# UM-ARM-Lab/pytorch_volumetric

Measured on AMD Instinct MI355X. Metric: SDF (val+grad) queries/sec, higher is better.
Workload: dtype f32

## Files before the change

pytorch_volumetric_amd/csrc/mesh.hip:

```cpp
#include "common.h"
#include "mesh_math.h"
#include "mesh_records.h"
#include "morton.h"
#include "order_small.h"
#include "wave_ops.h"

namespace pvamd {


struct MeshArgs {
    const float* normal;
    const float* rec;
    const float* tiles;
    const int* rec_of_face;
    int F;
    double ray_dir[3];
    unsigned long long* pairs;
};
#define PVAMD_COUNT_PAIRS(m, which, n)                                                                                  \
    do {                                                                                                                \
        if ((m).pairs) {                                                                                                \
            const unsigned long long count_ = (unsigned long long)(n);  \
            if ((int)(threadIdx.x & 63) == __builtin_ctzll(__ballot(true))) atomicAdd((m).pairs + (which), count_);     \
        }                                                                                                               \
// ... 94 lines not shown
        sx += __shfl_xor(sx, off, 64); sy += __shfl_xor(sy, off, 64);
        sz += __shfl_xor(sz, off, 64); sn += __shfl_xor(sn, off, 64);
    }
    if (lane == 0) { sh[wave][0] = sx; sh[wave][1] = sy; sh[wave][2] = sz; sh[wave][3] = sn; }
    __syncthreads();
    const float tn = sh[0][3] + sh[1][3] + sh[2][3] + sh[3][3];
    const float mx = (sh[0][0] + sh[1][0] + sh[2][0] + sh[3][0]) / tn;
    const float my = (sh[0][1] + sh[1][1] + sh[2][1] + sh[3][1]) / tn;
    const float mz = (sh[0][2] + sh[1][2] + sh[2][2] + sh[3][2]) / tn;
    __syncthreads();
    float reach = 0.f;
    if (live) {
        const float dx = cx - mx, dy = cy - my, dz = cz - mz;
        reach = sqrt_rn(dx * dx + dy * dy + dz * dz) * 1.00001f + r;
    }
    for (int off = 32; off > 0; off >>= 1) reach = fmaxf(reach, __shfl_xor(reach, off, 64));
    if (lane == 0) sh[wave][0] = reach;
    __syncthreads();
    if (threadIdx.x == 0) {
        float* w = tiles + 4 * (int64_t)tile;
        w[0] = mx; w[1] = my; w[2] = mz;
        w[3] = fmaxf(fmaxf(sh[0][0], sh[1][0]), fmaxf(sh[2][0], sh[3][0])) * 1.00001f + abs_margin;
    }
}

PVAMD_DEV float norm3_unfused(V3 g) {
    return sqrt_rn(add_rn(add_rn(mul_rn(g.x, g.x), mul_rn(g.y, g.y)), mul_rn(g.z, g.z)));
}

struct LaneState {
    V3 p;
    float reach;
    float reach2m, reach2x;
};

PVAMD_DEV void set_reach(LaneState& s, float reach) {
    s.reach = reach;
    s.reach2m = reach * reach * 1.00001f;
    s.reach2x = 2.00002f * reach;
}

PVAMD_DEV bool sphere_may_improve(const LaneState& s, float dist2, float r) {
    return !(dist2 > fmaf(r, fmaf(r, 1.00001f, s.reach2x), s.reach2m));
}

PVAMD_DEV bool sphere_may_hit(float dist2, float tp, float r) {
    const float perp2 = fmaf(-tp, tp, dist2);
    return !(perp2 > fmaf(r, r, 2e-6f * dist2)) && !(tp < -r);
}

PVAMD_DEV bool rect_may_improve(const LaneState& s, V3 w, float dist2, V3 fu, float hu, V3 fv, float hv, float m0) {
    const float u = dot(fu, w), v = dot(fv, w);
    const float h2 = fmaxf(fmaf(-v, v, fmaf(-u, u, dist2)), 0.f);
    const float du = fmaxf(fabsf(u) - hu, 0.f), dv = fmaxf(fabsf(v) - hv, 0.f);
    const float lb2 = fmaf(dv, dv, fmaf(du, du, h2));
    return !(lb2 > fmaf(8e-6f, dist2, s.reach2m + m0));
}

constexpr int kQueueCap = 128;
constexpr unsigned long long kBestInit = 0x7F80000000000000ull;

template <bool WITH_RAY>
struct WaveLocal {
    f32x4 sphere[64], fu[64], fv[64];
    float m0[64];
    unsigned qc[kQueueCap];
    unsigned qr[WITH_RAY ? kQueueCap : 1];
};
template <bool WITH_RAY>
struct GroupShared {
    unsigned long long best[64];
    int hits[WITH_RAY ? 64 : 1];
    int handed;
    float dir[WITH_RAY ? 192 : 1];
    float dn[WITH_RAY ? 192 : 1];
};
template <int SLICES, bool WITH_RAY>
struct MeshShared {
    GroupShared<WITH_RAY> g;
    WaveLocal<WITH_RAY> w[SLICES];
};

PVAMD_DEV float uniform(float v) { return __int_as_float(__builtin_amdgcn_readfirstlane(__float_as_int(v))); }

struct WaveBound {
    LaneState q;
    float rho;
    V3 dn0;
    float k, rho_k;
};

template <bool WITH_RAY>
struct Wave {
    LaneState s;
    bool live;
    V3 dn, dir;
    WaveBound wb;
    int nc, nr;
};

template <bool WITH_RAY>
PVAMD_DEV void refresh_bound(Wave<WITH_RAY>& wv) {
    const float rmax = wave_max(wv.live ? wv.s.reach : 0.f);
    set_reach(wv.wb.q, uniform((rmax + wv.wb.rho) * 1.00001f));
}

template <bool WITH_RAY>
PVAMD_DEV void pull_reach(const GroupShared<WITH_RAY>& g, Wave<WITH_RAY>& wv) {
    const float d2 = __int_as_float((int)(unsigned)(g.best[threadIdx.x & 63] >> 32));
    const float reach = fast_sqrt(d2) * 1.00001f + 1.1e-19f;
    if (reach < wv.s.reach) set_reach(wv.s, reach);
    refresh_bound(wv);
}

template <bool WITH_RAY>
PVAMD_DEV bool wave_setup(const MeshArgs& m, Wave<WITH_RAY>& wv) {
    const V3 p = wv.s.p;
    wv.live = fabsf(p.x) < INFINITY && fabsf(p.y) < INFINITY && fabsf(p.z) < INFINITY;
    wv.nc = wv.nr = 0;
    set_reach(wv.s, INFINITY);
    if (__ballot(wv.live) == 0ull) return false;
    const float lx = wave_min(wv.live ? p.x : INFINITY), hx = wave_max(wv.live ? p.x : -INFINITY);
    const float ly = wave_min(wv.live ? p.y : INFINITY), hy = wave_max(wv.live ? p.y : -INFINITY);
    const float lz = wave_min(wv.live ? p.z : INFINITY), hz = wave_max(wv.live ? p.z : -INFINITY);
    wv.wb.q.p = v3(uniform(0.5f * lx + 0.5f * hx), uniform(0.5f * ly + 0.5f * hy), uniform(0.5f * lz + 0.5f * hz));
    const V3 d = v3(p.x - wv.wb.q.p.x, p.y - wv.wb.q.p.y, p.z - wv.wb.q.p.z);
    wv.wb.rho = uniform(wave_max(wv.live ? fast_sqrt(dot(d, d)) : 0.f) * 1.00001f + 1.1e-19f);
    wv.wb.dn0 = v3(0.f, 0.f, 0.f);
    wv.wb.k = wv.wb.rho_k = 0.f;
    if (WITH_RAY) {
        const V3 a = v3((float)m.ray_dir[0], (float)m.ray_dir[1], (float)m.ray_dir[2]);
        const float inv = 1.f / sqrt_rn(dot(a, a));
        wv.wb.dn0 = v3(uniform(a.x * inv), uniform(a.y * inv), uniform(a.z * inv));
        const V3 e = v3(wv.dn.x - wv.wb.dn0.x, wv.dn.y - wv.wb.dn0.y, wv.dn.z - wv.wb.dn0.z);
        const float chord = wave_max(wv.live ? fast_sqrt(dot(e, e)) : 0.f);
        wv.wb.k = uniform(2.001f * chord + 2e-6f);
        wv.wb.rho_k = uniform(wv.wb.rho * (1.f + wv.wb.k) * 1.00001f);
    }
    set_reach(wv.wb.q, INFINITY);
    return true;
}

PVAMD_DEV bool axis_may_hit(const WaveBound& wb, V3 w, float dist2, float r) {
    const float dist = fast_sqrt(dist2) * 1.00001f + 1.1e-19f;
    return sphere_may_hit(dist2, dot(w, wb.dn0), fmaf(wb.k, dist, r + wb.rho_k));
}

PVAMD_DEV void enqueue(unsigned* q, int& n, unsigned long long mask, bool mine, int j) {
    const int lane = threadIdx.x & 63;
    if (mine) q[n + __popcll(mask & ((1ull << lane) - 1ull))] = ((unsigned)j << 6) | (unsigned)lane;
    n += __popcll(mask);
}

template <class Fn>
PVAMD_DEV void drain(unsigned* q, int& n, bool everything, Fn&& fn) {
    const int lane = threadIdx.x & 63;
    PVAMD_WAVE_SYNC();
    fn(n < 64 ? n : 64, q);
    if (n > 64) {
        const int rem = n - 64;
        if (everything) {
            fn(rem, q + 64);
            n = 0;
        } else {
            const unsigned v = lane < rem ? q[64 + lane] : 0u;
            if (lane < rem) q[lane] = v;
            n = rem;
        }
    } else {
        n = 0;
    }
    PVAMD_WAVE_SYNC();
}

template <bool WITH_RAY>
PVAMD_DEV void drain_closest(const MeshArgs& m, GroupShared<WITH_RAY>& g, WaveLocal<WITH_RAY>& wl, Wave<WITH_RAY>& wv, bool everything) {
    if (wv.nc == 0) return;
    const int lane = threadIdx.x & 63;
    drain(wl.qc, wv.nc, everything, [&](int count, const unsigned* q) {
        PVAMD_COUNT_PAIRS(m, 0, count);
        const unsigned e = lane < count ? q[lane] : 0u;
        const int owner = e & 63;
        const V3 p = v3(__shfl(wv.s.p.x, owner, 64), __shfl(wv.s.p.y, owner, 64), __shfl(wv.s.p.z, owner, 64));
        if (lane < count) {
            const int j = (int)(e >> 6);
            const f32x4 A = record_plane(m.rec, j, kPlaneA), B = record_plane(m.rec, j, kPlaneB), C = record_plane(m.rec, j, kPlaneC);
            const V3 qp = sub(closest_point_triangle(p, xyz(A), xyz(B), xyz(C)), p);
            const float d2 = dot(qp, qp);
            atomicMin(&g.best[owner], ((unsigned long long)(unsigned)__float_as_int(d2) << 32) | (unsigned)__float_as_int(A.w));
        }
    });
    pull_reach(g, wv);
}

template <bool WITH_RAY>
PVAMD_DEV void drain_rays(const MeshArgs& m, GroupShared<WITH_RAY>& g, WaveLocal<WITH_RAY>& wl, Wave<WITH_RAY>& wv, bool everything) {
    if (wv.nr == 0) return;
    const int lane = threadIdx.x & 63;
    drain(wl.qr, wv.nr, everything, [&](int count, const unsigned* q) {
        PVAMD_COUNT_PAIRS(m, 1, count);
        const unsigned e = lane < count ? q[lane] : 0u;
        const int owner = e & 63;
        const V3 p = v3(__shfl(wv.s.p.x, owner, 64), __shfl(wv.s.p.y, owner, 64), __shfl(wv.s.p.z, owner, 64));
        const V3 d = v3(__shfl(wv.dir.x, owner, 64), __shfl(wv.dir.y, owner, 64), __shfl(wv.dir.z, owner, 64));
        if (lane < count) {
            const int j = (int)(e >> 6);
            const f32x4 A = record_plane(m.rec, j, kPlaneA), B = record_plane(m.rec, j, kPlaneB), C = record_plane(m.rec, j, kPlaneC);
            if (ray_hits_triangle(p, d, xyz(A), xyz(B), xyz(C))) atomicAdd(&g.hits[owner], 1);
        }
    });
}

template <bool WITH_RAY>
PVAMD_DEV void visit_tile(const MeshArgs& m, GroupShared<WITH_RAY>& g, WaveLocal<WITH_RAY>& wl, Wave<WITH_RAY>& wv, int ti,
                          int pass_lo = 0, int pass_hi = kTile / 64) {
    const int lane = threadIdx.x & 63;
    const int ntiles = (m.F + kTile - 1) / kTile;
    const int n = min(kTile, m.F - ti * kTile);
    unsigned gm = 0u;
    {
        const bool gv = lane < kGroupsPerTile && lane * kGroup < n;
        const f32x4 gs = reinterpret_cast<const f32x4*>(m.tiles)[ntiles + ti * kGroupsPerTile + (gv ? lane : 0)];
        const V3 wc = v3(gs.x - wv.wb.q.p.x, gs.y - wv.wb.q.p.y, gs.z - wv.wb.q.p.z);
        const float dc2 = dot(wc, wc);
        bool coarse = sphere_may_improve(wv.wb.q, dc2, gs.w);
        if (WITH_RAY) coarse = coarse || axis_may_hit(wv.wb, wc, dc2, gs.w);
        unsigned todo = (unsigned)__ballot(coarse && gv);
        todo &= ((1u << (pass_hi * (64 / kGroup))) - 1u) & ~((1u << (pass_lo * (64 / kGroup))) - 1u);
        while (todo != 0u) {
            const int b = __builtin_ctz(todo);
            todo &= todo - 1u;
            const V3 ctr = v3(__int_as_float(__builtin_amdgcn_readlane(__float_as_int(gs.x), b)),
                              __int_as_float(__builtin_amdgcn_readlane(__float_as_int(gs.y), b)),
                              __int_as_float(__builtin_amdgcn_readlane(__float_as_int(gs.z), b)));
            const float r = __int_as_float(__builtin_amdgcn_readlane(__float_as_int(gs.w), b));
            const V3 w = v3(ctr.x - wv.s.p.x, ctr.y - wv.s.p.y, ctr.z - wv.s.p.z);
            const float dist2 = dot(w, w);
            bool need = sphere_may_improve(wv.s, dist2, r);
            if (WITH_RAY) need = need || sphere_may_hit(dist2, dot(w, wv.dn), r);
            if (__ballot(need && wv.live) != 0ull) gm |= 1u << b;
        }
    }
    const f32x4* P0 = tile_plane(m.rec, ti, kPlaneSphere);
    const f32x4* P1 = tile_plane(m.rec, ti, kPlaneU);
    const f32x4* P2 = tile_plane(m.rec, ti, kPlaneV);
    const f32x4* P4 = tile_plane(m.rec, ti, kPlaneB);
    for (int pass = pass_lo; pass < pass_hi; ++pass) {
        if (((gm >> (pass * (64 / kGroup))) & ((1u << (64 / kGroup)) - 1u)) == 0u) continue;
        const int idx = pass * 64 + lane;
        const f32x4 a0 = P0[idx], a1 = P1[idx], a2 = P2[idx];
        const float am0 = P4[idx].w;
        bool keep_c, keep_r = false;
        {
            const bool valid = idx < n && ((gm >> (idx / kGroup)) & 1u);
            const V3 w = v3(a0.x - wv.wb.q.p.x, a0.y - wv.wb.q.p.y, a0.z - wv.wb.q.p.z);
            const float dist2 = dot(w, w);
            keep_c = valid && sphere_may_improve(wv.wb.q, dist2, a0.w) &&
                     rect_may_improve(wv.wb.q, w, dist2, xyz(a1), a1.w, xyz(a2), a2.w, am0);
            if (WITH_RAY) keep_r = valid && axis_may_hit(wv.wb, w, dist2, a0.w);
        }
        const unsigned long long mc = __ballot(keep_c), mr = WITH_RAY ? __ballot(keep_r) : 0ull;
        unsigned long long todo = mc | mr;
        if (todo == 0ull) continue;
        PVAMD_WAVE_SYNC();
        wl.sphere[lane] = a0;
        wl.fu[lane] = a1;
        wl.fv[lane] = a2;
        wl.m0[lane] = am0;
        PVAMD_WAVE_SYNC();
        const int j0 = ti * kTile + pass * 64;
        const unsigned long long live_mask = __ballot(wv.live);
        while (todo != 0ull) {
            const int b = __builtin_ctzll(todo);
            todo &= todo - 1ull;
            const f32x4 o = wl.sphere[b];
            const V3 w = v3(o.x - wv.s.p.x, o.y - wv.s.p.y, o.z - wv.s.p.z);
            const float dist2 = dot(w, w);
            if (!WITH_RAY || ((mc >> b) & 1ull)) {
                const unsigned long long near_c = live_mask & __ballot(sphere_may_improve(wv.s, dist2, o.w));
                if (near_c != 0ull) {
                    const f32x4 u = wl.fu[b], v = wl.fv[b];
                    const unsigned long long mk = near_c & __ballot(rect_may_improve(wv.s, w, dist2, xyz(u), u.w, xyz(v), v.w, wl.m0[b]));
                    if (mk) {
                        enqueue(wl.qc, wv.nc, mk, __builtin_amdgcn_inverse_ballot_w64(mk), j0 + b);
                        if (wv.nc >= 64) drain_closest(m, g, wl, wv, false);
                    }
                }
            }
            if (WITH_RAY && ((mr >> b) & 1ull)) {
                const unsigned long long mk = live_mask & __ballot(sphere_may_hit(dist2, dot(w, wv.dn), o.w));
                if (mk) {
                    enqueue(wl.qr, wv.nr, mk, __builtin_amdgcn_inverse_ballot_w64(mk), j0 + b);
                    if (wv.nr >= 64) drain_rays(m, g, wl, wv, false);
                }
            }
        }
    }
}

template <bool WITH_RAY>
PVAMD_DEV int scan_seed(const MeshArgs& m, Wave<WITH_RAY>& wv, int part, int nparts) {
    const int lane = threadIdx.x & 63;
    const int ntiles = (m.F + kTile - 1) / kTile;
    const f32x4* tiles4 = reinterpret_cast<const f32x4*>(m.tiles);
    float bound = INFINITY, own = INFINITY;
    int nearest = -1;
    for (int base = 0; base < ntiles; base += 64) {
        const int ti = base + lane;
        if (ti < ntiles) {
            const f32x4 ts = tiles4[ti];
            const V3 w = v3(ts.x - wv.wb.q.p.x, ts.y - wv.wb.q.p.y, ts.z - wv.wb.q.p.z);
            const float b = fast_sqrt(dot(w, w)) * 1.00001f + (ts.w + 1.1e-19f);
            bound = fminf(bound, b);
            if ((nparts == 1 || (ti % nparts) == part) && (b < own || nearest < 0)) {
                own = b < own ? b : own;
                nearest = ti;
            }
        }
    }
    const float lowest = wave_min(bound);
    set_reach(wv.s, (lowest + wv.wb.rho) * 1.00001f);
    refresh_bound(wv);
    const float mine = wave_min(own);
    unsigned long long at = __ballot(nearest >= 0 && own == mine);
    if (at == 0ull) at = __ballot(nearest >= 0);
    return at ? __builtin_amdgcn_readlane(nearest, __builtin_ctzll(at)) : -1;
}

template <bool WITH_RAY>
PVAMD_DEV void greedy_reach(const MeshArgs& m, GroupShared<WITH_RAY>& g, Wave<WITH_RAY>& wv, int ti) {
    const int ntiles = (m.F + kTile - 1) / kTile;
    const f32x4* spheres = reinterpret_cast<const f32x4*>(m.tiles);
    const V3 p = wv.s.p;
    auto reach_of = [&](f32x4 sp) {
        const V3 w = v3(sp.x - p.x, sp.y - p.y, sp.z - p.z);
        return fast_sqrt(dot(w, w)) * 1.00001f + (sp.w + 1.1e-19f);
    };
    float bound = INFINITY;
    int gi = 0;
    const int ngroups = (min(kTile, m.F - ti * kTile) + kGroup - 1) / kGroup;
    for (int k = 0; k < ngroups; ++k) {
        const float b = reach_of(spheres[ntiles + ti * kGroupsPerTile + k]);
        if (b < bound) { bound = b; gi = k; }
    }
    const int j0 = ti * kTile + gi * kGroup;
    float nearest = INFINITY;
    int jn = -1;
    for (int k = 0; k < kGroup; ++k) {
        if (j0 + k < m.F) {
            const float b = reach_of(record_plane(m.rec, j0 + k, kPlaneSphere));
            if (b < nearest) { nearest = b; jn = j0 + k; }
        }
    }
    PVAMD_COUNT_PAIRS(m, 0, __popcll(__ballot(jn >= 0 && wv.live)));
    if (jn >= 0 && wv.live) {
        const f32x4 A = record_plane(m.rec, jn, kPlaneA), B = record_plane(m.rec, jn, kPlaneB), C = record_plane(m.rec, jn, kPlaneC);
        const V3 qp = sub(closest_point_triangle(p, xyz(A), xyz(B), xyz(C)), p);
        const float d2 = dot(qp, qp);
        atomicMin(&g.best[threadIdx.x & 63], ((unsigned long long)(unsigned)__float_as_int(d2) << 32) | (unsigned)__float_as_int(A.w));
    }
    bound = fminf(bound, nearest) * 1.00001f;
    if (bound < wv.s.reach) set_reach(wv.s, bound);
    pull_reach(g, wv);
}

template <bool WITH_RAY>
PVAMD_DEV void scan_tiles(const MeshArgs& m, GroupShared<WITH_RAY>& g, WaveLocal<WITH_RAY>& wl, Wave<WITH_RAY>& wv, int skip,
                          int part, int nparts, int pass_lo = 0, int pass_hi = kTile / 64) {
    const int lane = threadIdx.x & 63;
    const int ntiles = (m.F + kTile - 1) / kTile;
    const f32x4* tiles4 = reinterpret_cast<const f32x4*>(m.tiles);
    for (int base = 0; base < ntiles; base += 64) {
        const int ti = base + lane;
        const bool mine = ti < ntiles && ti != skip && (nparts == 1 || (ti % nparts) == part);
        const f32x4 ts = tiles4[mine ? ti : 0];
        const V3 w = v3(ts.x - wv.wb.q.p.x, ts.y - wv.wb.q.p.y, ts.z - wv.wb.q.p.z);
        const float dist2 = dot(w, w);
        const bool ray = WITH_RAY && mine && axis_may_hit(wv.wb, w, dist2, ts.w);
        const float lower = mine ? fast_sqrt(dist2) - ts.w : INFINITY;
        unsigned long long done = 0ull;
        for (;;) {
            pull_reach(g, wv);
            const bool need = mine && (ray || sphere_may_improve(wv.wb.q, dist2, ts.w));
            const unsigned long long todo = __ballot(need) & ~done;
            if (todo == 0ull) break;
            const float key = ((todo >> lane) & 1ull) ? lower : INFINITY;
            const unsigned long long at = __ballot(key == wave_min(key)) & todo;
            const int t = __builtin_ctzll(at ? at : todo);
            done |= 1ull << t;
            const V3 ctr = v3(__int_as_float(__builtin_amdgcn_readlane(__float_as_int(ts.x), t)),
                              __int_as_float(__builtin_amdgcn_readlane(__float_as_int(ts.y), t)),
                              __int_as_float(__builtin_amdgcn_readlane(__float_as_int(ts.z), t)));
            const float r = __int_as_float(__builtin_amdgcn_readlane(__float_as_int(ts.w), t));
            const V3 wl_ = v3(ctr.x - wv.s.p.x, ctr.y - wv.s.p.y, ctr.z - wv.s.p.z);
            const float d2 = dot(wl_, wl_);
            bool mine_too = sphere_may_improve(wv.s, d2, r);
            if (WITH_RAY) mine_too = mine_too || sphere_may_hit(d2, dot(wl_, wv.dn), r);
            if (__ballot(mine_too && wv.live) == 0ull) continue;
            visit_tile<WITH_RAY>(m, g, wl, wv, base + t, pass_lo, pass_hi);
        }
    }
}

template <bool WITH_RAY>
PVAMD_DEV void scan_finish(const MeshArgs& m, GroupShared<WITH_RAY>& g, WaveLocal<WITH_RAY>& wl, Wave<WITH_RAY>& wv) {
    drain_closest(m, g, wl, wv, true);
    if (WITH_RAY) drain_rays(m, g, wl, wv, true);
}

template <bool WITH_RAY>
PVAMD_DEV bool scan_begin(const MeshArgs& m, GroupShared<WITH_RAY>& g, Wave<WITH_RAY>& wv, int wave, uint64_t seed,
                          int64_t jitter_index, const unsigned long long* start, const float* __restrict__ drawn = nullptr,
                          const float* __restrict__ bound = nullptr) {
    const int lane = threadIdx.x & 63;
    if (wave == 0) {
        g.best[lane] = start ? *start : kBestInit;
        if (WITH_RAY) {
            g.hits[lane] = 0;
            const V3 dir = drawn ? v3(drawn[3 * lane], drawn[3 * lane + 1], drawn[3 * lane + 2])
                                 : jitter_dir(m.ray_dir, seed, jitter_index);
            const float inv_len = 1.f / sqrt_rn(dot(dir, dir));
            g.dir[3 * lane] = dir.x; g.dir[3 * lane + 1] = dir.y; g.dir[3 * lane + 2] = dir.z;
            g.dn[3 * lane] = dir.x * inv_len; g.dn[3 * lane + 1] = dir.y * inv_len; g.dn[3 * lane + 2] = dir.z * inv_len;
        }
    }
    __syncthreads();
    wv.dir = wv.dn = v3(0.f, 0.f, 0.f);
    if (WITH_RAY) {
        wv.dir = v3(g.dir[3 * lane], g.dir[3 * lane + 1], g.dir[3 * lane + 2]);
        wv.dn = v3(g.dn[3 * lane], g.dn[3 * lane + 1], g.dn[3 * lane + 2]);
    }
    return bound ? load_bound(bound, wv) : wave_setup(m, wv);
}

struct HandOver {
    int* count;
    int* entries;
    unsigned long long* best;
    int* hits;
    float* dir;
    float* reach;
    float* pts;
    unsigned long long* p_best;
    float* p_dir;
    float* p_reach;
    float* bound;
    int cap;
};
constexpr int kBoundFloats = 16;
constexpr int kSmallPoints = PVAMD_MESH_SMALL_POINTS;
static_assert(PVAMD_MESH_SMALL_POINTS <= kOrderSmallPoints, "an unordered query is sorted by ONE workgroup (order_small_block), which drops the points beyond its capacity");
constexpr int kHandOverHeader = 64;
struct HandOverLayout {
    size_t entries, best, hits, dir, reach, bound, pts;
    size_t p_best, p_dir, p_reach;
    size_t bytes;
};
constexpr HandOverLayout hand_over_layout(int64_t cap) {
    const size_t slots = (size_t)cap, lanes = slots * 64, small = (size_t)kSmallPoints;
    HandOverLayout l = {};
    l.entries = kHandOverHeader;
    l.best = l.entries + slots * 2 * sizeof(int);
    l.hits = l.best + lanes * sizeof(unsigned long long);
    l.dir = l.hits + lanes * sizeof(int);
    l.reach = l.dir + lanes * 3 * sizeof(float);
    l.bound = l.reach + lanes * sizeof(float);
    l.pts = l.bound + slots * kBoundFloats * sizeof(float);
    l.p_best = l.pts + lanes * 3 * sizeof(float);
    l.p_dir = l.p_best + small * sizeof(unsigned long long);
    l.p_reach = l.p_dir + small * 3 * sizeof(float);
    l.bytes = l.p_reach + small * sizeof(float);
    return l;
}
static_assert(hand_over_layout(PVAMD_MESH_SCRATCH_SLOTS(0)).bytes == PVAMD_MESH_SCRATCH_BYTES(0) &&
              hand_over_layout(PVAMD_MESH_SCRATCH_SLOTS(1)).bytes == PVAMD_MESH_SCRATCH_BYTES(1),
              "PVAMD_MESH_SCRATCH_BYTES is not the hand-over layout's total");
static_assert(hand_over_layout(0).bytes - hand_over_layout(0).p_best == (size_t)kSmallPoints * (sizeof(unsigned long long) + 4 * sizeof(float)),
              "the by-point part holds one (best, dir, reach) per point of the largest unordered query");

static HandOver hand_over(void* scratch, int cap) {
    const HandOverLayout l = hand_over_layout(cap);
    char* base = reinterpret_cast<char*>(scratch);
    HandOver h;
    h.count = reinterpret_cast<int*>(base);
    h.entries = reinterpret_cast<int*>(base + l.entries);
    h.best = reinterpret_cast<unsigned long long*>(base + l.best);
    h.hits = reinterpret_cast<int*>(base + l.hits);
    h.dir = reinterpret_cast<float*>(base + l.dir);
    h.reach = reinterpret_cast<float*>(base + l.reach);
    h.bound = reinterpret_cast<float*>(base + l.bound);
    h.pts = reinterpret_cast<float*>(base + l.pts);
    h.p_best = reinterpret_cast<unsigned long long*>(base + l.p_best);
    h.p_dir = reinterpret_cast<float*>(base + l.p_dir);
    h.p_reach = reinterpret_cast<float*>(base + l.p_reach);
    h.cap = scratch ? cap : 0;
    return h;
}
constexpr int kHeavy32nds = 6;
constexpr int kHeavyMinTiles = 128;
constexpr int kHeavyParts = 32;

PVAMD_DEV void store_bound(float* __restrict__ b, const WaveBound& wb, bool any_live) {
    if ((threadIdx.x & 63) != 0) return;
    b[0] = wb.q.p.x; b[1] = wb.q.p.y; b[2] = wb.q.p.z; b[3] = wb.rho;
    b[4] = wb.dn0.x; b[5] = wb.dn0.y; b[6] = wb.dn0.z; b[7] = wb.k;
    b[8] = wb.rho_k; b[9] = any_live ? 1.f : 0.f;
    b[10] = wb.q.reach;
}
template <bool WITH_RAY>
PVAMD_DEV bool part_has_work(const MeshArgs& m, const float* __restrict__ b, int part, int nparts) {
    if (uniform(b[9]) == 0.f) return false;
    WaveBound wb;
    wb.q.p = v3(uniform(b[0]), uniform(b[1]), uniform(b[2]));
    wb.rho = uniform(b[3]);
    wb.dn0 = v3(uniform(b[4]), uniform(b[5]), uniform(b[6]));
    wb.k = uniform(b[7]);
    wb.rho_k = uniform(b[8]);
    set_reach(wb.q, uniform(b[10]));
    const int lane = threadIdx.x & 63;
    const int ntiles = (m.F + kTile - 1) / kTile;
    const f32x4* tiles4 = reinterpret_cast<const f32x4*>(m.tiles);
    for (int base = part; base < ntiles; base += 64 * nparts) {
        const int ti = base + lane * nparts;
        const f32x4 ts = tiles4[ti < ntiles ? ti : 0];
        const V3 w = v3(ts.x - wb.q.p.x, ts.y - wb.q.p.y, ts.z - wb.q.p.z);
        const float dist2 = dot(w, w);
        bool need = sphere_may_improve(wb.q, dist2, ts.w);
        if (WITH_RAY) need = need || axis_may_hit(wb, w, dist2, ts.w);
        if (__ballot(need && ti < ntiles) != 0ull) return true;
    }
    return false;
}
template <bool WITH_RAY>
PVAMD_DEV bool load_bound(const float* __restrict__ b, Wave<WITH_RAY>& wv) {
    const V3 p = wv.s.p;
    wv.live = fabsf(p.x) < INFINITY && fabsf(p.y) < INFINITY && fabsf(p.z) < INFINITY;
    wv.nc = wv.nr = 0;
    set_reach(wv.s, INFINITY);
    wv.wb.q.p = v3(uniform(b[0]), uniform(b[1]), uniform(b[2]));
    wv.wb.rho = uniform(b[3]);
    wv.wb.dn0 = v3(uniform(b[4]), uniform(b[5]), uniform(b[6]));
    wv.wb.k = uniform(b[7]);
    wv.wb.rho_k = uniform(b[8]);
    set_reach(wv.wb.q, INFINITY);
    return uniform(b[9]) != 0.f;
}

template <bool WITH_RAY>
PVAMD_DEV int flagged_tiles(const MeshArgs& m, const Wave<WITH_RAY>& wv) {
    const int lane = threadIdx.x & 63;
    const int ntiles = (m.F + kTile - 1) / kTile;
    const f32x4* tiles4 = reinterpret_cast<const f32x4*>(m.tiles);
// ... 182 lines not shown
    const int ntiles = (m.F + kTile - 1) / kTile;
    const f32x4* spheres = reinterpret_cast<const f32x4*>(m.tiles);
    auto reach_of = [&](f32x4 sp) {
        const V3 w = v3(sp.x - p.x, sp.y - p.y, sp.z - p.z);
        return fast_sqrt(dot(w, w)) * 1.00001f + (sp.w + 1.1e-19f);
    };
    int ti = 0;
    for (int base = 0; base < ntiles; base += 64) {
        const f32x4 mine = spheres[base + lane < ntiles ? base + lane : base];
        const int n = min(64, ntiles - base);
        for (int t = 0; t < n; ++t) {
            const f32x4 sp = {__int_as_float(__builtin_amdgcn_readlane(__float_as_int(mine.x), t)),
                              __int_as_float(__builtin_amdgcn_readlane(__float_as_int(mine.y), t)),
                              __int_as_float(__builtin_amdgcn_readlane(__float_as_int(mine.z), t)),
                              __int_as_float(__builtin_amdgcn_readlane(__float_as_int(mine.w), t))};
            const float b = reach_of(sp);
            if (b < bound) { bound = b; ti = base + t; }
        }
    }
    int gi = 0;
    const int ngroups = (min(kTile, m.F - ti * kTile) + kGroup - 1) / kGroup;
    for (int k = 0; k < kGroupsPerTile; ++k) {
        if (k >= ngroups) break;
        const float b = reach_of(spheres[ntiles + ti * kGroupsPerTile + k]);
        if (b < bound) { bound = b; gi = k; }
    }
    const int j0 = ti * kTile + gi * kGroup;
    float nearest = INFINITY;
    int jn = -1;
    for (int k = 0; k < kGroup; ++k) {
        if (j0 + k >= m.F) break;
        const float b = reach_of(record_plane(m.rec, j0 + k, kPlaneSphere));
        if (b < nearest) { nearest = b; jn = j0 + k; }
    }
    bound = fminf(bound, nearest);
    PVAMD_COUNT_PAIRS(m, 0, __popcll(__ballot(jn >= 0 && fabsf(p.x) < INFINITY && fabsf(p.y) < INFINITY && fabsf(p.z) < INFINITY)));
    if (jn >= 0 && fabsf(p.x) < INFINITY && fabsf(p.y) < INFINITY && fabsf(p.z) < INFINITY) {
        const f32x4 A = record_plane(m.rec, jn, kPlaneA), B = record_plane(m.rec, jn, kPlaneB), C = record_plane(m.rec, jn, kPlaneC);
        const V3 qp = sub(closest_point_triangle(p, xyz(A), xyz(B), xyz(C)), p);
        const float d2 = dot(qp, qp);
        found = ((unsigned long long)(unsigned)__float_as_int(d2) << 32) | (unsigned)__float_as_int(A.w);
        if (!(found < kBestInit)) found = kBestInit;
        else bound = fminf(bound, fast_sqrt(d2) * 1.00001f + 1.1e-19f);
    }
    return bound * 1.00001f;
}

__global__ __launch_bounds__(128) void hand_over_all_kernel(MeshArgs m, const int* __restrict__ order, const float* __restrict__ pts,
                                                            int64_t P, uint64_t seed, int64_t index_base, HandOver ho, int groups) {
    __shared__ float reach_of_lane[64];
    const int g = blockIdx.x, lane = threadIdx.x & 63;
    const int64_t slot = (int64_t)g * 64 + lane;
    const int64_t i = point_index(order, slot, P);
    if (threadIdx.x < 64) {
        ho.hits[slot] = 0;
        const V3 dir = jitter_dir(m.ray_dir, seed, index_base + i);
        float* o = ho.dir + slot * 3;
        o[0] = dir.x; o[1] = dir.y; o[2] = dir.z;
        {
            Wave<true> wv{};
            wv.s.p = v3(pts[3 * i], pts[3 * i + 1], pts[3 * i + 2]);
            const float inv_len = 1.f / sqrt_rn(dot(dir, dir));
            wv.dir = dir;
            wv.dn = v3(dir.x * inv_len, dir.y * inv_len, dir.z * inv_len);
            const bool any_live = wave_setup(m, wv);
            float* q = ho.pts + slot * 3;
            q[0] = wv.s.p.x; q[1] = wv.s.p.y; q[2] = wv.s.p.z;
            if (lane == 0) {
                ho.entries[2 * g] = g;
                ho.entries[2 * g + 1] = 0;
                if (g == 0) *ho.count = groups;
            }
            __syncthreads();
            if (any_live) {
                set_reach(wv.s, reach_of_lane[lane]);
                refresh_bound(wv);
            }
            store_bound(ho.bound + (int64_t)g * kBoundFloats, wv.wb, any_live);
        }
        return;
    }
    unsigned long long found;
    const float bound = greedy_bound(m, v3(pts[3 * i], pts[3 * i + 1], pts[3 * i + 2]), found);
    ho.best[slot] = found;
    ho.reach[slot] = bound;
    reach_of_lane[lane] = bound;
    __syncthreads();
}
__global__ void hand_over_none_kernel(HandOver ho) { *ho.count = 0; }

constexpr int kPrepPoints = 512;
static unsigned small_prep_blocks(int64_t P) { return 1 + (unsigned)((P + kPrepPoints - 1) / kPrepPoints); }
static_assert(kOrderSmallThreads == 1024 && kPrepPoints * 2 == kOrderSmallThreads,
              "mesh_small_prep_kernel: block 0 runs order_small_block, the others 512 points on two halves of 1024 threads");
__global__ __launch_bounds__(1024) void mesh_small_prep_kernel(MeshArgs m, const float* __restrict__ pts, int P, uint64_t seed,
                                                               int64_t index_base, int* __restrict__ order, HandOver ho) {
    if (blockIdx.x == 0) {
        order_small_block(pts, P, order, nullptr, nullptr);
        return;
    }
    const int wave = threadIdx.x >> 6, lane = threadIdx.x & 63;
    const int i = ((int)blockIdx.x - 1) * kPrepPoints + (wave & 7) * 64 + lane;
    const int ii = i < P ? i : P - 1;
    if (((int)blockIdx.x - 1) * kPrepPoints + (wave & 7) * 64 >= P) return;
    if (wave < 8) {
        const V3 dir = jitter_dir(m.ray_dir, seed, index_base + ii);
        if (i < P) {
            float* o = ho.p_dir + 3 * (int64_t)i;
            o[0] = dir.x; o[1] = dir.y; o[2] = dir.z;
        }
    } else {
        unsigned long long found;
        const float bound = greedy_bound(m, v3(pts[3 * ii], pts[3 * ii + 1], pts[3 * ii + 2]), found);
        if (i < P) {
            ho.p_best[i] = found;
            ho.p_reach[i] = bound;
        }
    }
}

__global__ __launch_bounds__(64) void hand_over_gather_kernel(MeshArgs m, const int* __restrict__ order, const float* __restrict__ pts,
                                                              int64_t P, HandOver ho, int groups) {
    const int g = blockIdx.x, lane = threadIdx.x;
    const int64_t slot = (int64_t)g * 64 + lane;
    const int64_t i = point_index(order, slot, P);
    const V3 dir = v3(ho.p_dir[3 * i], ho.p_dir[3 * i + 1], ho.p_dir[3 * i + 2]);
    const float reach = ho.p_reach[i];
    ho.best[slot] = ho.p_best[i];
    ho.reach[slot] = reach;
    ho.hits[slot] = 0;
    float* o = ho.dir + slot * 3;
    o[0] = dir.x; o[1] = dir.y; o[2] = dir.z;
    Wave<true> wv{};
    wv.s.p = v3(pts[3 * i], pts[3 * i + 1], pts[3 * i + 2]);
    float* q = ho.pts + slot * 3;
    q[0] = wv.s.p.x; q[1] = wv.s.p.y; q[2] = wv.s.p.z;
    const float inv_len = 1.f / sqrt_rn(dot(dir, dir));
    wv.dir = dir;
    wv.dn = v3(dir.x * inv_len, dir.y * inv_len, dir.z * inv_len);
    const bool any_live = wave_setup(m, wv);
    if (any_live) {
        set_reach(wv.s, reach);
        refresh_bound(wv);
    }
    store_bound(ho.bound + (int64_t)g * kBoundFloats, wv.wb, any_live);
    if (lane == 0) {
        ho.entries[2 * g] = g;
        ho.entries[2 * g + 1] = 0;
        if (g == 0) *ho.count = groups;
    }
}

constexpr int kPartsMinWaves = 7;
template <bool WITH_RAY, bool WAIT = false, int WAVES = kTile / 64>
PVAMD_DEV void parts_of_group(const MeshArgs& m, MeshShared<WAVES, WITH_RAY>& sh, uint64_t seed, const HandOver& ho, int slot) {
    const int lane = threadIdx.x & 63, wave = __builtin_amdgcn_readfirstlane(threadIdx.x >> 6);
    if (!part_has_work<WITH_RAY>(m, ho.bound + (int64_t)slot * kBoundFloats, (int)blockIdx.y, (int)gridDim.y)) return;
    Wave<WITH_RAY> wv;
    const float* q = ho.pts + ((int64_t)slot * 64 + lane) * 3;
    wv.s.p = v3(q[0], q[1], q[2]);
    const unsigned long long start = ho.best[(int64_t)slot * 64 + lane];
    const float known = ho.reach[(int64_t)slot * 64 + lane];
    if (scan_begin(m, sh.g, wv, wave, seed, 0, &start, WITH_RAY ? ho.dir + (int64_t)slot * 192 : nullptr,
                   ho.bound + (int64_t)slot * kBoundFloats)) {
        if (__any(wv.live && !(known < INFINITY) && (unsigned)(start >> 32) >= 0x7F800000u)) scan_seed(m, wv, 0, 1);
        if (known < wv.s.reach) set_reach(wv.s, known);
        refresh_bound(wv);
        constexpr int kPasses = (kTile / 64) / WAVES;
        scan_tiles<WITH_RAY>(m, sh.g, sh.w[wave], wv, -1, (int)blockIdx.y, (int)gridDim.y, wave * kPasses, (wave + 1) * kPasses);
        scan_finish(m, sh.g, sh.w[wave], wv);
    }
    __syncthreads();
    if (wave == 0) {
        if (WAIT) {
            unsigned long long was = 0ull;
            int had = 0;
            if (sh.g.best[lane] < start) was = atomicMin(&ho.best[(int64_t)slot * 64 + lane], sh.g.best[lane]);
            if (WITH_RAY && sh.g.hits[lane] != 0) had = atomicAdd(&ho.hits[(int64_t)slot * 64 + lane], sh.g.hits[lane]);
            asm volatile("" ::"v"(was), "v"(had) : "memory");
        } else {
            if (sh.g.best[lane] < start) atomicMin(&ho.best[(int64_t)slot * 64 + lane], sh.g.best[lane]);
            if (WITH_RAY && sh.g.hits[lane] != 0) atomicAdd(&ho.hits[(int64_t)slot * 64 + lane], sh.g.hits[lane]);
        }
    }
}

template <int kAllWaves>
__global__ __launch_bounds__(64 * kAllWaves, kPartsMinWaves) void mesh_parts_all_kernel(MeshArgs m, const int* __restrict__ order,
                                                                          const float* __restrict__ pts, int64_t P,
                                                                          uint64_t seed, HandOver ho, QueryOut out) {
    __shared__ __attribute__((aligned(16))) MeshShared<kAllWaves, true> sh;
    const int g = (int)blockIdx.x;
    parts_of_group<true, true, kAllWaves>(m, sh, seed, ho, g);
    if (threadIdx.x >= 64) return;
    const int lane = threadIdx.x;
    int done = 0;
    if (lane == 0) done = atomicAdd(&ho.entries[2 * g + 1], 1);
    if (__builtin_amdgcn_readfirstlane(done) != (int)gridDim.y - 1) return;
    const int64_t k = (int64_t)g * 64 + lane;
    if (k >= P) return;
    const int64_t i = order ? (int64_t)order[k] : k;
    const unsigned long long found = atomicMin(&ho.best[k], ~0ull);
    const int hits = atomicOr(&ho.hits[k], 0);
    write_query(m, out, i, v3(pts[3 * i], pts[3 * i + 1], pts[3 * i + 2]), found, hits);
}

template <bool WITH_RAY, int WAVES>
__global__ __launch_bounds__(64 * WAVES, kPartsMinWaves) void mesh_parts_kernel(MeshArgs m, uint64_t seed, HandOver ho) {
    __shared__ __attribute__((aligned(16))) MeshShared<WAVES, WITH_RAY> sh;
    const int listed = min(*ho.count, ho.cap);
    for (int slot = blockIdx.x; slot < listed; slot += gridDim.x) {
        parts_of_group<WITH_RAY, false, WAVES>(m, sh, seed, ho, slot);
        __syncthreads();
    }
}

__global__ __launch_bounds__(64) void mesh_query_finish_kernel(MeshArgs m, const int* __restrict__ order,
                                                               const float* __restrict__ pts, int64_t P, HandOver ho,
                                                               QueryOut out) {
    const int listed = min(*ho.count, ho.cap);
    for (int slot = blockIdx.x; slot < listed; slot += gridDim.x) {
        const int64_t k = (int64_t)ho.entries[2 * slot] * 64 + threadIdx.x;
        if (k >= P) continue;
        const int64_t i = order ? (int64_t)order[k] : k;
        write_query(m, out, i, v3(pts[3 * i], pts[3 * i + 1], pts[3 * i + 2]), ho.best[(int64_t)slot * 64 + threadIdx.x],
                    ho.hits[(int64_t)slot * 64 + threadIdx.x]);
    }
}

__global__ __launch_bounds__(64) void chamfer_finish_kernel(MeshArgs m, const int* __restrict__ order, const float* __restrict__ W,
                                                            const float* __restrict__ pts, int64_t N, float scale, HandOver ho,
                                                            double* __restrict__ out_sum, int64_t per) {
    const int listed = min(*ho.count, ho.cap);
    for (int slot = blockIdx.x; slot < listed; slot += gridDim.x) {
        const int64_t k = (int64_t)ho.entries[2 * slot] * 64 + threadIdx.x;
        const int b = ho.entries[2 * slot + 1];
        const int64_t i = point_index(order, k, N);
        const V3 p = W ? chamfer_point(W + 16 * (int64_t)b, pts, i) : v3(pts[3 * i], pts[3 * i + 1], pts[3 * i + 2]);
        chamfer_accumulate(m, p, k < N, ho.best[(int64_t)slot * 64 + threadIdx.x], scale, W ? out_sum + b : out_sum, i, W ? 0 : per);
    }
}

__global__ __launch_bounds__(256) void morton_keys_kernel(const float* __restrict__ pts, int64_t P,
                                                          const float* __restrict__ box, int* __restrict__ keys) {
    const int64_t i = (int64_t)blockIdx.x * blockDim.x + threadIdx.x;
    if (i >= P) return;
    const float lo[3] = {box[0], box[1], box[2]}, hi[3] = {box[3], box[4], box[5]};
    keys[i] = (int)morton_key30(pts[3 * i], pts[3 * i + 1], pts[3 * i + 2], lo, hi);
}

__global__ void aabb_init_kernel(unsigned* box) {
    if (threadIdx.x < 3) box[threadIdx.x] = order_code(INFINITY);
    else if (threadIdx.x < 6) box[threadIdx.x] = order_code(-INFINITY);
}
__global__ __launch_bounds__(256) void aabb_reduce_kernel(const float* __restrict__ pts, int64_t P, unsigned* box) {
    float lo[3] = {INFINITY, INFINITY, INFINITY}, hi[3] = {-INFINITY, -INFINITY, -INFINITY};
    for (int64_t i = (int64_t)blockIdx.x * blockDim.x + threadIdx.x; i < P; i += (int64_t)gridDim.x * blockDim.x) {
#pragma unroll
        for (int d = 0; d < 3; ++d) {
            const float v = pts[3 * i + d];
            if (fabsf(v) < INFINITY) {
                lo[d] = fminf(lo[d], v);
                hi[d] = fmaxf(hi[d], v);
            }
        }
    }
#pragma unroll
    for (int d = 0; d < 3; ++d) {
        for (int off = 32; off > 0; off >>= 1) {
            lo[d] = fminf(lo[d], __shfl_xor(lo[d], off, 64));
            hi[d] = fmaxf(hi[d], __shfl_xor(hi[d], off, 64));
        }
    }
    __shared__ float part[4][6];
    const int wave = threadIdx.x >> 6, lane = threadIdx.x & 63;
    if (lane == 0) {
#pragma unroll
        for (int d = 0; d < 3; ++d) { part[wave][d] = lo[d]; part[wave][3 + d] = hi[d]; }
    }
    __syncthreads();
    if (threadIdx.x < 3) {
        const int d = threadIdx.x;
        atomicMin(box + d, order_code(fminf(fminf(part[0][d], part[1][d]), fminf(part[2][d], part[3][d]))));
    } else if (threadIdx.x < 6) {
        const int d = threadIdx.x;
        atomicMax(box + d, order_code(fmaxf(fmaxf(part[0][d], part[1][d]), fmaxf(part[2][d], part[3][d]))));
    }
}
__global__ void aabb_decode_kernel(unsigned* box) {
    if (threadIdx.x < 6) reinterpret_cast<float*>(box)[threadIdx.x] = order_decode(box[threadIdx.x]);
}

__global__ void zero_f64_kernel(double* p, int n) {
    const int i = blockIdx.x * blockDim.x + threadIdx.x;
    if (i < n) p[i] = 0.0;
}

__global__ void invert_face_order_kernel(const float* __restrict__ rec, int F, int* __restrict__ rec_of_face) {
    const int k = blockIdx.x * blockDim.x + threadIdx.x;
    if (k < F) rec_of_face[__float_as_int(record_plane(rec, k, kPlaneA).w)] = k;
}

static MeshArgs mesh_args(const pvamd_mesh_t& mesh) {
    MeshArgs m;
    m.normal = mesh.normal;
    m.rec = mesh.rec;
    m.tiles = mesh.tiles;
    m.rec_of_face = mesh.rec_of_face;
    m.F = mesh.F;
    for (int d = 0; d < 3; ++d) m.ray_dir[d] = mesh.ray_dir[d];
    m.pairs = reinterpret_cast<unsigned long long*>(mesh.pair_counters);
    return m;
}

constexpr int kMaxFaces = 1 << 26;

__global__ __launch_bounds__(256) void grid_points_kernel(const float* __restrict__ cx, const float* __restrict__ cy,
                                                          const float* __restrict__ cz, int nx, int ny, int nz,
                                                          float* __restrict__ pts, int* __restrict__ order) {
    const int64_t n = (int64_t)nx * ny * nz;
    const int64_t i = (int64_t)blockIdx.x * blockDim.x + threadIdx.x;
    if (i >= n) return;
    const int z = (int)(i % nz), y = (int)((i / nz) % ny), x = (int)(i / ((int64_t)nz * ny));
    pts[3 * i] = cx[x];
    pts[3 * i + 1] = cy[y];
    pts[3 * i + 2] = cz[z];
    const int Bx = x >> 4, By = y >> 4, Bz = z >> 4;
    const int Wx = min(16, nx - 16 * Bx), Wy = min(16, ny - 16 * By), Wz = min(16, nz - 16 * Bz);
    const int sx = x & 15, sy = y & 15, sz = z & 15;
    const int bx = sx >> 2, by = sy >> 2, bz = sz >> 2;
    const int wx = min(4, Wx - 4 * bx), wy = min(4, Wy - 4 * by), wz = min(4, Wz - 4 * bz);
    const int64_t j = (int64_t)(16 * Bx) * ny * nz + (int64_t)Wx * (16 * By) * nz + (int64_t)Wx * Wy * (16 * Bz) +
                      ((int64_t)(4 * bx) * Wy * Wz + (int64_t)wx * (4 * by) * Wz + (int64_t)wx * wy * (4 * bz)) +
                      ((int64_t)((sx & 3) * wy + (sy & 3)) * wz + (sz & 3));
    order[j] = (int)i;
}

using MeshPlan = pvamd_mesh_plan_t;
constexpr int kMaxSlices = 8;
constexpr int kMinParts = 4;
constexpr int kHeavyPartWaves = 4;
constexpr int kWideScanOverTiles = 128;

static int scan_waves_for(int64_t groups, int ntiles, bool hands_over) {
    int s = 2;
    while (s < 8 && (int64_t)s * groups < 16384) s <<= 1;
    if (ntiles > kWideScanOverTiles && !hands_over) s = 8;
    if (s > kMaxSlices) s = kMaxSlices;
    while (s > 1 && s > ntiles) s >>= 1;
    return s;
}

static void plan_scan(MeshPlan& pl, int64_t rows, int ntiles, bool has_scratch) {
    const bool hands_over = has_scratch && ntiles >= kHeavyMinTiles;
    pl.path = hands_over ? PVAMD_MESH_PATH_SCAN_HEAVY : PVAMD_MESH_PATH_SCAN;
    pl.scan_waves = scan_waves_for(pl.groups * rows, ntiles, hands_over);
    pl.parts = hands_over ? (kHeavyParts < ntiles ? kHeavyParts : ntiles) : 0;
    pl.part_waves = hands_over ? kHeavyPartWaves : 0;
}

static MeshPlan mesh_query_plan(int64_t P, int F, bool has_scratch, bool unordered) {
    MeshPlan pl = {};
    const int64_t groups = (P + 63) / 64;
    const int ntiles = (F + kTile - 1) / kTile;
    pl.groups = (int32_t)groups;
// ... 227 lines not shown
```

Baseline: 213.2 billion.

## Add point-serial traversal mode for tile passes in mesh_parts_kernel

Adds a POINT_SERIAL variant of visit_tile. When few query points want a tile pass compared with the number of surviving triangles, it loops over those points and tests all triangles in parallel across lanes, instead of looping over triangles and testing all points. Candidate records are enqueued with the point index so the existing closest-point and ray drains can process them. The mode is enabled only in mesh_parts_kernel and adds extra ballots and readlanes per point in exchange for better lane utilisation when points are sparse.

After: 210.1 billion. 0.986x the previous value.

```diff
diff --git a/pytorch_volumetric_amd/csrc/mesh.hip b/pytorch_volumetric_amd/csrc/mesh.hip
--- a/pytorch_volumetric_amd/csrc/mesh.hip
+++ b/pytorch_volumetric_amd/csrc/mesh.hip
@@ -270,6 +270,15 @@
     n += __popcll(mask);
 }
 
+PVAMD_DEV void enqueue_records(unsigned* q, int& n, unsigned long long mask, int j0, int i) {
+    const int lane = threadIdx.x & 63;
+    if ((mask >> lane) & 1ull) q[n + __popcll(mask & ((1ull << lane) - 1ull))] = ((unsigned)(j0 + lane) << 6) | (unsigned)i;
+    n += __popcll(mask);
+}
+
+constexpr int kPointSerialA = 1, kPointSerialB = 1;
+constexpr bool point_serial_pays(int points, int survivors) { return points * kPointSerialA < survivors * kPointSerialB; }
+
 template <class Fn>
 PVAMD_DEV void drain(unsigned* q, int& n, bool everything, Fn&& fn) {
     const int lane = threadIdx.x & 63;
@@ -329,13 +338,14 @@
     });
 }
 
-template <bool WITH_RAY>
+template <bool WITH_RAY, bool POINT_SERIAL = false>
 PVAMD_DEV void visit_tile(const MeshArgs& m, GroupShared<WITH_RAY>& g, WaveLocal<WITH_RAY>& wl, Wave<WITH_RAY>& wv, int ti,
                           int pass_lo = 0, int pass_hi = kTile / 64) {
     const int lane = threadIdx.x & 63;
     const int ntiles = (m.F + kTile - 1) / kTile;
     const int n = min(kTile, m.F - ti * kTile);
     unsigned gm = 0u;
+    unsigned mine_g = 0u;
     {
         const bool gv = lane < kGroupsPerTile && lane * kGroup < n;
         const f32x4 gs = reinterpret_cast<const f32x4*>(m.tiles)[ntiles + ti * kGroupsPerTile + (gv ? lane : 0)];
@@ -357,6 +367,7 @@
             bool need = sphere_may_improve(wv.s, dist2, r);
             if (WITH_RAY) need = need || sphere_may_hit(dist2, dot(w, wv.dn), r);
             if (__ballot(need && wv.live) != 0ull) gm |= 1u << b;
+            if (POINT_SERIAL) mine_g |= (need && wv.live) ? 1u << b : 0u;
         }
     }
     const f32x4* P0 = tile_plane(m.rec, ti, kPlaneSphere);
@@ -380,6 +391,48 @@
         const unsigned long long mc = __ballot(keep_c), mr = WITH_RAY ? __ballot(keep_r) : 0ull;
         unsigned long long todo = mc | mr;
         if (todo == 0ull) continue;
+        if (POINT_SERIAL) {
+            unsigned long long points = __ballot(((mine_g >> (pass * (64 / kGroup))) & ((1u << (64 / kGroup)) - 1u)) != 0u);
+            if (point_serial_pays(__popcll(points), __popcll(todo))) {
+                const int j0 = ti * kTile + pass * 64;
+                const unsigned my_group = 1u << (idx / kGroup);
+                const V3 ctr = xyz(a0);
+                while (points != 0ull) {
+                    const int i = __builtin_ctzll(points);
+                    points &= points - 1ull;
+                    LaneState s;
+                    s.p = v3(__int_as_float(__builtin_amdgcn_readlane(__float_as_int(wv.s.p.x), i)),
+                             __int_as_float(__builtin_amdgcn_readlane(__float_as_int(wv.s.p.y), i)),
+                             __int_as_float(__builtin_amdgcn_readlane(__float_as_int(wv.s.p.z), i)));
+                    s.reach = 0.f;
+                    s.reach2m = __int_as_float(__builtin_amdgcn_readlane(__float_as_int(wv.s.reach2m), i));
+                    s.reach2x = __int_as_float(__builtin_amdgcn_readlane(__float_as_int(wv.s.reach2x), i));
+                    const unsigned groups_i = (unsigned)__builtin_amdgcn_readlane((int)mine_g, i);
+                    const unsigned long long wanted = __ballot((groups_i & my_group) != 0u);
+                    const V3 w = v3(ctr.x - s.p.x, ctr.y - s.p.y, ctr.z - s.p.z);
+                    const float dist2 = dot(w, w);
+                    const unsigned long long near_c = mc & wanted & __ballot(sphere_may_improve(s, dist2, a0.w));
+                    if (near_c != 0ull) {
+                        const unsigned long long mk = near_c & __ballot(rect_may_improve(s, w, dist2, xyz(a1), a1.w, xyz(a2), a2.w, am0));
+                        if (mk) {
+                            enqueue_records(wl.qc, wv.nc, mk, j0, i);
+                            if (wv.nc >= 64) drain_closest(m, g, wl, wv, false);
+                        }
+                    }
+                    if (WITH_RAY && (mr & wanted) != 0ull) {
+                        const V3 dn = v3(__int_as_float(__builtin_amdgcn_readlane(__float_as_int(wv.dn.x), i)),
+                                         __int_as_float(__builtin_amdgcn_readlane(__float_as_int(wv.dn.y), i)),
+                                         __int_as_float(__builtin_amdgcn_readlane(__float_as_int(wv.dn.z), i)));
+                        const unsigned long long mk = mr & wanted & __ballot(sphere_may_hit(dist2, dot(w, dn), a0.w));
+                        if (mk) {
+                            enqueue_records(wl.qr, wv.nr, mk, j0, i);
+                            if (wv.nr >= 64) drain_rays(m, g, wl, wv, false);
+                        }
+                    }
+                }
+                continue;
+            }
+        }
         PVAMD_WAVE_SYNC();
         wl.sphere[lane] = a0;
         wl.fu[lane] = a1;
@@ -482,7 +535,7 @@
     pull_reach(g, wv);
 }
 
-template <bool WITH_RAY>
+template <bool WITH_RAY, bool POINT_SERIAL = false>
 PVAMD_DEV void scan_tiles(const MeshArgs& m, GroupShared<WITH_RAY>& g, WaveLocal<WITH_RAY>& wl, Wave<WITH_RAY>& wv, int skip,
                           int part, int nparts, int pass_lo = 0, int pass_hi = kTile / 64) {
     const int lane = threadIdx.x & 63;
@@ -515,7 +568,7 @@
             bool mine_too = sphere_may_improve(wv.s, d2, r);
             if (WITH_RAY) mine_too = mine_too || sphere_may_hit(d2, dot(wl_, wv.dn), r);
             if (__ballot(mine_too && wv.live) == 0ull) continue;
-            visit_tile<WITH_RAY>(m, g, wl, wv, base + t, pass_lo, pass_hi);
+            visit_tile<WITH_RAY, POINT_SERIAL>(m, g, wl, wv, base + t, pass_lo, pass_hi);
         }
     }
 }
@@ -1004,7 +1057,7 @@
 }
 
 constexpr int kPartsMinWaves = 7;
-template <bool WITH_RAY, bool WAIT = false, int WAVES = kTile / 64>
+template <bool WITH_RAY, bool WAIT, int WAVES, bool POINT_SERIAL>
 PVAMD_DEV void parts_of_group(const MeshArgs& m, MeshShared<WAVES, WITH_RAY>& sh, uint64_t seed, const HandOver& ho, int slot) {
     const int lane = threadIdx.x & 63, wave = __builtin_amdgcn_readfirstlane(threadIdx.x >> 6);
     if (!part_has_work<WITH_RAY>(m, ho.bound + (int64_t)slot * kBoundFloats, (int)blockIdx.y, (int)gridDim.y)) return;
@@ -1019,7 +1072,7 @@
         if (known < wv.s.reach) set_reach(wv.s, known);
         refresh_bound(wv);
         constexpr int kPasses = (kTile / 64) / WAVES;
-        scan_tiles<WITH_RAY>(m, sh.g, sh.w[wave], wv, -1, (int)blockIdx.y, (int)gridDim.y, wave * kPasses, (wave + 1) * kPasses);
+        scan_tiles<WITH_RAY, POINT_SERIAL>(m, sh.g, sh.w[wave], wv, -1, (int)blockIdx.y, (int)gridDim.y, wave * kPasses, (wave + 1) * kPasses);
         scan_finish(m, sh.g, sh.w[wave], wv);
     }
     __syncthreads();
@@ -1043,7 +1096,7 @@
                                                                           uint64_t seed, HandOver ho, QueryOut out) {
     __shared__ __attribute__((aligned(16))) MeshShared<kAllWaves, true> sh;
     const int g = (int)blockIdx.x;
-    parts_of_group<true, true, kAllWaves>(m, sh, seed, ho, g);
+    parts_of_group<true, true, kAllWaves, false>(m, sh, seed, ho, g);
     if (threadIdx.x >= 64) return;
     const int lane = threadIdx.x;
     int done = 0;
@@ -1062,7 +1115,7 @@
     __shared__ __attribute__((aligned(16))) MeshShared<WAVES, WITH_RAY> sh;
     const int listed = min(*ho.count, ho.cap);
     for (int slot = blockIdx.x; slot < listed; slot += gridDim.x) {
-        parts_of_group<WITH_RAY, false, WAVES>(m, sh, seed, ho, slot);
+        parts_of_group<WITH_RAY, false, WAVES, true>(m, sh, seed, ho, slot);
         __syncthreads();
     }
 }
```
